# mmammel8/kmer_id

Measured on AMD Instinct MI355X. Metric: paired reads classified/sec on bact10 DB, higher is better.
Workload: dtype u64

## Files before the change

include/kmer_id_amd_bench.h:

```cpp
#ifndef KMER_ID_AMD_BENCH_H
#define KMER_ID_AMD_BENCH_H
#include <stdint.h>
#ifdef __cplusplus
extern "C" {
#endif
struct kid_db;
struct kid_sample;
int kid_synth_db_keys_host(uint64_t seed, int k, const uint64_t *cum, int32_t ntar,
                           uint64_t j0, uint64_t n, uint64_t *keys, uint32_t *targets);
int kid_synth_db_keys_device(uint64_t seed, int k, const uint64_t *cum_host, int32_t ntar,
                             uint64_t j0, uint64_t n, void *d_keys, void *d_targets, int device);
int kid_synth_reads_host(uint64_t db_seed, uint64_t read_seed, int k, const uint64_t *cum,
                         const int32_t *parent, int32_t ntar, uint64_t r0, uint64_t n_reads,
                         uint32_t read_len, uint8_t *bases);
int kid_synth_reads_device(uint64_t db_seed, uint64_t read_seed, int k, const uint64_t *cum_host,
                           const int32_t *parent_host, int32_t ntar, uint64_t r0, uint64_t n_reads,
                           uint32_t read_len, void *d_bases, int device);

int kid_bench_gather(struct kid_db *db, uint64_t n_loads, int inflight, int iters, float *ms_out, uint64_t *loads_out);

int kid_sample_kernel_variants(struct kid_sample *s, uint64_t *mask);

int kid_sample_log_state(struct kid_sample *s, uint32_t *passes, int *has_log, int *logging);

int kid_dev_alloc(int device, uint64_t nbytes, void **d_ptr);
int kid_dev_free(int device, void *d_ptr);
int kid_dev_upload(int device, void *d_dst, const void *src, uint64_t nbytes);
int kid_dev_download(int device, void *dst, const void *d_src, uint64_t nbytes);
int kid_dev_sync(int device);

#ifdef __cplusplus
}
#endif
#endif
```

kmer_id_amd/_lib.py:

```python
import ctypes as C
import os

from . import _build

c_u8p = C.POINTER(C.c_uint8)
c_u32p = C.POINTER(C.c_uint32)
c_i32p = C.POINTER(C.c_int32)
c_u64p = C.POINTER(C.c_uint64)
c_i64p = C.POINTER(C.c_int64)
c_void_pp = C.POINTER(C.c_void_p)


class KidDbInfo(C.Structure):
    _fields_ = [
        ("ntar", C.c_int32), ("k", C.c_int32), ("log2_slots", C.c_int32), ("max_probes", C.c_int32),
        ("flags", C.c_uint32), ("device", C.c_int32), ("tree_depth", C.c_int32), ("host_built", C.c_int32),
        ("geometry", C.c_int32), ("reserved_", C.c_int32),
        ("n_entries", C.c_uint64), ("n_occupied", C.c_uint64), ("table_bytes", C.c_uint64),
    ]


PROTOTYPES = {
    "kid_strerror": (C.c_char_p, [C.c_int]),
    "kid_last_error": (C.c_char_p, []),
# ... 47 lines not shown
    "kid_db_read_segments_fastq": (C.c_int, [C.c_void_p, C.c_void_p, C.c_uint64, C.c_void_p, C.c_uint64, C.c_uint32, C.c_uint32,
                                             C.c_uint32, C.c_uint32, C.c_void_p, C.c_void_p, C.c_uint64, c_u64p]),
    "kid_db_read_segments_device": (C.c_int, [C.c_void_p, C.c_void_p, C.c_uint64, C.c_void_p, C.c_void_p, C.c_void_p, C.c_uint64,
                                              C.c_uint32, C.c_uint32, C.c_uint32, C.c_uint32, C.c_void_p, C.c_uint64, C.c_void_p,
                                              C.c_void_p, C.c_uint64, C.c_void_p, C.c_void_p, C.c_void_p]),
    "kid_db_read_segments_time": (C.c_int, [C.c_void_p, C.POINTER(C.c_double), c_u64p, c_u64p]),
    "kid_sample_end": (C.c_int, [C.c_void_p, C.c_void_p, C.c_void_p]),
    "kid_sample_end_merged": (C.c_int, [c_void_pp, C.c_int, C.c_void_p, C.c_void_p]),
    "kid_sample_stats": (C.c_int, [C.c_void_p, C.c_void_p]),
    "kid_sample_set_timing": (C.c_int, [C.c_void_p, C.c_int]),
    "kid_sample_kernel_time": (C.c_int, [C.c_void_p, C.POINTER(C.c_double), c_u64p]),
    "kid_sample_kernel_time_device": (C.c_int, [C.c_void_p, C.POINTER(C.c_double), c_u64p]),
    "kid_sample_seen_bytes": (C.c_int, [C.c_void_p, c_u64p]),
    "kid_sample_seen_export": (C.c_int, [C.c_void_p, C.c_uint64, C.c_uint64, C.c_void_p, C.c_int]),
    "kid_sample_seen_or": (C.c_int, [C.c_void_p, C.c_uint64, C.c_uint64, C.c_void_p, C.c_int]),
    "kid_sample_gcount": (C.c_int, [C.c_void_p, C.c_void_p]),
    "kid_sample_ucount_range": (C.c_int, [C.c_void_p, C.c_uint64, C.c_uint64, C.c_void_p]),
    "kid_sample_depth_export": (C.c_int, [C.c_void_p, C.c_uint64, C.c_uint64, C.c_void_p, C.c_int]),
    "kid_sample_depth_add": (C.c_int, [C.c_void_p, C.c_uint64, C.c_uint64, C.c_void_p, C.c_int]),
    "kid_sample_depth_spectrum": (C.c_int, [C.c_void_p, C.c_uint32, C.c_void_p, C.c_void_p, C.c_void_p]),
    "kid_sample_depth_spectrum_merged": (C.c_int, [c_void_pp, C.c_int, C.c_uint32, C.c_void_p, C.c_void_p, C.c_void_p]),
    "kid_db_shared_kmers": (C.c_int, [C.c_void_p, c_void_pp, C.c_int, C.c_int, C.c_void_p]),
    "kid_shared_kmers": (C.c_int, [C.c_int, C.c_void_p, C.c_uint64, C.c_int32, c_void_pp, C.c_int, C.c_int, C.c_void_p]),
    "kid_shared_kmers_time": (C.c_int, [C.POINTER(C.c_double), c_u64p]),
    "kid_synth_db_keys_host": (C.c_int, [C.c_uint64, C.c_int, C.c_void_p, C.c_int32, C.c_uint64, C.c_uint64, C.c_void_p,
                                         C.c_void_p]),
    "kid_synth_db_keys_device": (C.c_int, [C.c_uint64, C.c_int, C.c_void_p, C.c_int32, C.c_uint64, C.c_uint64, C.c_void_p,
                                           C.c_void_p, C.c_int]),
    "kid_synth_reads_host": (C.c_int, [C.c_uint64, C.c_uint64, C.c_int, C.c_void_p, C.c_void_p, C.c_int32, C.c_uint64,
                                       C.c_uint64, C.c_uint32, C.c_void_p]),
    "kid_synth_reads_device": (C.c_int, [C.c_uint64, C.c_uint64, C.c_int, C.c_void_p, C.c_void_p, C.c_int32, C.c_uint64,
                                         C.c_uint64, C.c_uint32, C.c_void_p, C.c_int]),
    "kid_sample_kernel_variants": (C.c_int, [C.c_void_p, c_u64p]),
    "kid_sample_log_state": (C.c_int, [C.c_void_p, c_u32p, C.POINTER(C.c_int), C.POINTER(C.c_int)]),
    "kid_bench_gather": (C.c_int, [C.c_void_p, C.c_uint64, C.c_int, C.c_int, C.POINTER(C.c_float), c_u64p]),
    "kid_dev_alloc": (C.c_int, [C.c_int, C.c_uint64, c_void_pp]),
    "kid_dev_free": (C.c_int, [C.c_int, C.c_void_p]),
    "kid_dev_upload": (C.c_int, [C.c_int, C.c_void_p, C.c_void_p, C.c_uint64]),
    "kid_dev_download": (C.c_int, [C.c_int, C.c_void_p, C.c_void_p, C.c_uint64]),
    "kid_dev_sync": (C.c_int, [C.c_int]),
    "kid_device_mem_info": (C.c_int, [C.c_int, c_u64p, c_u64p]),
    "kid_builder_create": (C.c_int, [C.c_int, C.c_int, C.c_void_p, C.c_int32, C.c_uint64, c_void_pp]),
    "kid_builder_destroy": (None, [C.c_void_p]),
    "kid_builder_add": (C.c_int, [C.c_void_p, C.c_void_p, C.c_uint64, C.c_int32]),
    "kid_builder_remove": (C.c_int, [C.c_void_p, C.c_void_p, C.c_uint64]),
    "kid_builder_set_minct": (C.c_int, [C.c_void_p, C.c_void_p, C.c_int32]),
    "kid_builder_claim": (C.c_int, [C.c_void_p, C.c_void_p, C.c_uint64, C.c_int64, C.c_void_p, C.c_uint64, c_u64p]),
    "kid_builder_size": (C.c_int, [C.c_void_p, c_u64p]),
    "kid_builder_export": (C.c_int, [C.c_void_p, C.c_uint64, C.c_uint64, C.c_void_p]),
    "kid_builder_entropy": (C.c_int, [C.c_void_p, C.c_void_p, C.c_uint64, C.c_void_p]),
    "kid_builder_stats": (C.c_int, [C.c_void_p, C.c_void_p, C.c_void_p]),
}

KID_OPT_INPUTS_READY = 1
KID_OPT_LONG_RECORD_KMERS = 2
KID_OPT_MIN_BASE_QUALITY = 3
KID_OPT_ENTRY_DEPTH = 4
KID_DB_OPT_MIN_BASE_QUALITY = 1
KID_SHARED_MAX_SAMPLES = 64
KID_FLAG_U_IS_T = 1
KID_FLAG_HOST_BUILD = 2
KID_FLAG_REF_GEOMETRY = 4

_lib = None


# ... 45 lines not shown
```

kmer_id_amd/api.py:

```python
import ctypes as C
import struct

import numpy as np

from . import _lib
from ._lib import KidDbInfo, check


def _ptr(a):
    return a.ctypes.data_as(C.c_void_p) if a is not None else None


def _as(a, dtype):
    if a is None:
        return None
    a = np.ascontiguousarray(a, dtype=dtype)
    return a


def _offsets_batch(bases, offsets, start, stop):
    offsets = _as(offsets, np.uint64)
    return _as(bases, np.uint8), offsets, _as(start, np.int32), _as(stop, np.int32), offsets.size - 1


# ... 428 lines not shown
    def gcount(self):
        g = np.empty(self.ntar, np.int64)
        check(self._lib.kid_sample_gcount(self._h, _ptr(g)))
        return g

    def ucount_range(self, slot_begin, slot_end):
        u = np.empty(self.ntar, np.int64)
        check(self._lib.kid_sample_ucount_range(self._h, slot_begin, slot_end, _ptr(u)))
        return u

    def stats(self):
        out = np.zeros(4, np.uint64)
        check(self._lib.kid_sample_stats(self._h, _ptr(out)))
        return {"reads": int(out[0]), "lookups": int(out[1]), "probes": int(out[2]), "hits": int(out[3])}

    def set_timing(self, enabled=True):
        check(self._lib.kid_sample_set_timing(self._h, 1 if enabled else 0))

    def kernel_time(self):
        ms, n = C.c_double(0), C.c_uint64(0)
        check(self._lib.kid_sample_kernel_time(self._h, C.byref(ms), C.byref(n)))
        return ms.value, n.value

    def kernel_time_device(self):
        ms, n = C.c_double(0), C.c_uint64(0)
        check(self._lib.kid_sample_kernel_time_device(self._h, C.byref(ms), C.byref(n)))
        return ms.value, n.value

    def kernel_variants(self):
        m = C.c_uint64(0)
        check(self._lib.kid_sample_kernel_variants(self._h, C.byref(m)))
        return {(b >> 3 & 1, b >> 2 & 1, b >> 1 & 1, 30 if b & 1 else 0, b >> 4) for b in range(64) if m.value >> b & 1}

    def log_state(self):
        passes, has_log, logging = C.c_uint32(0), C.c_int(0), C.c_int(0)
        check(self._lib.kid_sample_log_state(self._h, C.byref(passes), C.byref(has_log), C.byref(logging)))
        return {"passes": passes.value, "has_log": bool(has_log.value), "logging": bool(logging.value)}

    def seen_bytes(self):
        n = C.c_uint64(0)
        check(self._lib.kid_sample_seen_bytes(self._h, C.byref(n)))
        return n.value

    def seen_export(self, byte_off, nbytes, dst_ptr=None, on_device=False):
        if dst_ptr is None:
            buf = np.empty(nbytes, np.uint8)
            check(self._lib.kid_sample_seen_export(self._h, byte_off, nbytes, _ptr(buf), 0))
            return buf
        check(self._lib.kid_sample_seen_export(self._h, byte_off, nbytes, C.c_void_p(dst_ptr), 1 if on_device else 0))
        return None

    def seen_or(self, byte_off, src, nbytes=None, on_device=False):
        if isinstance(src, np.ndarray):
            src = np.ascontiguousarray(src, np.uint8)
            check(self._lib.kid_sample_seen_or(self._h, byte_off, src.size, _ptr(src), 0))
        else:
            check(self._lib.kid_sample_seen_or(self._h, byte_off, nbytes, C.c_void_p(src), 1 if on_device else 0))

    def depth_spectrum(self, bins=256):
        spectrum, ksum, dmax = np.empty((self.ntar, bins), np.uint64), np.empty(self.ntar, np.uint64), np.empty(self.ntar, np.uint32)
        check(self._lib.kid_sample_depth_spectrum(self._h, bins, _ptr(spectrum), _ptr(ksum), _ptr(dmax)))
        return spectrum, ksum, dmax

    def entry_depth(self, begin=0, end=None):
        if end is None:
            end = self.db.info.n_entries
# ... 19 lines not shown
```

kmer_id_amd/csrc/kid_api.hip:

```cpp
#include <hip/hip_runtime.h>
#include <memory>
#include <stdint.h>
#include <string.h>
#include <type_traits>
#include <utility>
#include <vector>

#include "../../include/kmer_id_amd.h"
#include "kid_kernels.hip.h"
#include "kid_build.hip.h"
#include "kid_tile.hip.h"
#include "kid_long.hip.h"
#include "kid_hits.hip.h"
#include "kid_support.hip.h"
#include "kid_segments.hip.h"
#include "kid_mask.hip.h"
#include "kid_depth.hip.h"
#include "kid_shared.hip.h"
#include "kid_api_core.h"
#include "kid_api_db.h"
#include "kid_api_mask.h"
#include "kid_api_hits.h"
#include "kid_api_builder.h"
#include "kid_api_bench.h"
// ... 17 lines not shown
        KidDevBuf long_list;
        KidDevBuf long_plan;
        KidDevBuf rare;
        KidEvent ev_prep;
        KidEvent ev_used;
        hipStream_t used_stream = nullptr;
        bool used_recorded = false;
        bool used = false;
    };
    static const int NSET = 3;
    Scratch sets[NSET];
    uint32_t next_set = 0;
    bool inputs_ready = false;
    int min_base_quality = 0;
    KidDevBuf masked;
    int64_t long_kmers = 65536;
    KidDevBuf rare_fixed;
    struct { uint32_t *out_final = nullptr; uint64_t read0 = 0; uint32_t fixed_len = 0; int32_t fixed_nk = 0; bool valid = false; } fixed_held;
    uint64_t dev_clock_batches = 0;
    KidDevBuf seen_log, seen_log_tail, seen_sorted, log_counts, log_bin_total;
    uint32_t seen_log_cap = 0, log_nbins = 0;
    KidMappedHost log_host_total;
    bool log_dirty = false;
    bool log_off = false;
    uint32_t passes_done = 0;
    uint32_t launches_since_apply = 0;
    uint64_t reads_since_apply = 0;
    double log_entries_per_read = 4.0;
    uint64_t reads_of_last_pass = 0;
    KidDevBuf long_hits, long_tiles;
    bool ended = false;
    uint64_t reads_submitted = 0;
    uint64_t kernel_variants = 0;
    hipStream_t last_stream = nullptr;
    bool has_last_stream = false;
    KidEvent order_ev;
    struct Slot {
        KidDevBuf bases;
        KidDevBuf offsets, start, stop, out;
        KidDevBuf recs;
        KidEvent ev_h2d, ev_done, ev_out;
        std::vector<uint64_t> rel;
        uint64_t ticket = 0;
        bool busy = false;
    };
    static const int NSLOT = 3;
    Slot slots[NSLOT];
    uint64_t next_ticket = 1;

    unsigned long long *stats_p() const { return stats.as<unsigned long long>(); }
    volatile unsigned long long *log_rate() const { return static_cast<volatile unsigned long long *>(log_host_total.p); }
    volatile unsigned int *log_off_flag() const { return reinterpret_cast<volatile unsigned int *>(static_cast<char *>(log_host_total.p) + 8); }
};

extern "C" void kid_sample_destroy(kid_sample *s)
{
    if (!s) return;
    if (s->db) hipSetDevice(s->db->device);
    hipDeviceSynchronize();
    delete s;
}

static int kid_seenlog_point(kid_sample *s, hipStream_t stream);
extern "C" int kid_sample_reset(kid_sample *s)
{
    if (!s) return kid_fail(KID_ERR_ARG, "null sample");
    int rc = kid_use_device(s->db->device);
    if (rc != KID_OK) return rc;
    KID_HIP(hipDeviceSynchronize());
    const size_t nt = (size_t)s->db->info.ntar;
    KID_HIP(hipMemset(s->gcount.p, 0, nt * 8));
    KID_HIP(hipMemset(s->ucount.p, 0, nt * 8));
    KID_HIP(hipMemset(s->stats.p, 0, 256));
    KID_HIP(hipMemset(s->masked.p, 0, 8));
    {
        const unsigned long long never = ~0ull;
        KID_HIP(hipMemcpy(s->stats_p() + 30, &never, 8, hipMemcpyHostToDevice));
    }
    s->dev_clock_batches = 0;
    s->reads_submitted = 0;
    s->ended = false;
    s->kernel_variants = 0;
    if (s->seen_log_tail.p) KID_HIP(hipMemset(s->seen_log_tail.p, 0, KID_LOG_SHARDS * 64));
    if (s->seen_log.p) {
        int rc = kid_seenlog_point(s, nullptr);
        if (rc != KID_OK) return rc;
        *s->log_off_flag() = 0;
        *s->log_rate() = 0;
        s->log_off = false;
        s->passes_done = 0;
        s->log_entries_per_read = 4.0;
    }
    s->log_dirty = false;
    s->launches_since_apply = 0;
    s->reads_since_apply = 0;
    KID_HIP(hipMemset(s->seen.p, 0, s->seen_words * 4));
    if (s->depth.p) KID_HIP(hipMemset(s->depth.p, 0, s->seen_words * 32 * 4));
    KID_HIP(hipDeviceSynchronize());
    return KID_OK;
}

extern "C" int kid_sample_begin(kid_db *db, kid_sample **out)
{
    if (!db || !out) return kid_fail(KID_ERR_ARG, "null argument");
    *out = nullptr;
    int rc = kid_use_device(db->device);
    if (rc != KID_OK) return rc;
    std::unique_ptr<kid_sample, void (*)(kid_sample *)> s(new kid_sample(), kid_sample_destroy);
    s->db = db;
    const size_t nt = (size_t)db->info.ntar;
    s->seen_words = db->seen_bits / 32;
    KID_HIP(s->gcount.alloc(nt * 8));
    KID_HIP(s->ucount.alloc(nt * 8));
    KID_HIP(s->stats.alloc(256));
    KID_HIP(s->masked.alloc(8));
    KID_HIP(s->seen.alloc(s->seen_words * 4));
    KID_HIP(s->stream.create());
    const uint64_t nbins = (db->seen_bits + (1ull << KID_LOG_BIN_BITS) - 1) >> KID_LOG_BIN_BITS;
    if (db->d.minloc && nbins <= 1024) {
        uint64_t total = db->info.n_entries * 2ull;
        if (total < (32ull << 20)) total = 32ull << 20;
        if (total > (128ull << 20)) total = 128ull << 20;
        uint64_t cap = (total / KID_LOG_SHARDS) & ~63ull;
        s->seen_log_cap = (uint32_t)cap;
        s->log_nbins = (uint32_t)nbins;
        KID_HIP(s->seen_log.alloc(cap * KID_LOG_SHARDS * 4));
        KID_HIP(s->seen_sorted.alloc(cap * KID_LOG_SHARDS * 4));
        KID_HIP(s->seen_log_tail.alloc(KID_LOG_SHARDS * 64));
        KID_HIP(s->log_counts.alloc(nbins * KID_LOG_WGS * 4));
        KID_HIP(s->log_bin_total.alloc(nbins * 4));
        KID_HIP(s->log_host_total.alloc(64, hipHostMallocMapped));
        memset(s->log_host_total.p, 0, 64);
    }
    const KidRareArgs ra{s->gcount.as<unsigned long long>(), s->stats_p(), db->d.line_mask, 0u, 0ull, 0ull, 0, 0u, db->d.rows,
                         s->seen.as<uint32_t>(), nullptr, nullptr, s->seen_log.as<uint32_t>(), s->seen_log_tail.as<uint32_t>(),
                         s->seen_log_cap, 0u};
    for (kid_sample::Scratch &sc : s->sets) {
        KID_HIP(sc.rare.alloc(sizeof(ra)));
        KID_HIP(hipMemcpy(sc.rare.p, &ra, sizeof(ra), hipMemcpyHostToDevice));
        KID_HIP(sc.ev_prep.create(hipEventDisableTiming));
        KID_HIP(sc.ev_used.create(hipEventDisableTiming));
    }
    KID_HIP(s->rare_fixed.alloc(sizeof(ra)));
    KID_HIP(hipMemcpy(s->rare_fixed.p, &ra, sizeof(ra), hipMemcpyHostToDevice));
    rc = kid_sample_reset(s.get());
    if (rc != KID_OK) return rc;
    *out = s.release();
// ... 129 lines not shown
        }
        if (sc.used && sc.used_stream != prep_stream) {
            if (sc.used_recorded || hipEventRecord(sc.ev_used.e, sc.used_stream) == hipSuccess) KID_HIP(hipStreamWaitEvent(prep_stream, sc.ev_used.e, 0));
            else {
                (void)hipGetLastError();
                KID_HIP(hipDeviceSynchronize());
            }
        }
        const bool fuse_rebase = prep_stream == stream;
        if (fastq)
            hipLaunchKernelGGL(kid_prepare_fastq_kernel, dim3(kid_grid_for(b.n, 256, db->num_cu * 8)), dim3(256), 0, prep_stream, b.bases,
                               fastq, b.n, db->info.k, desc, const_cast<int32_t *>(b.start), const_cast<int32_t *>(b.stop),
                               b.out_final, stats, gcount, rare, ++s->batch_seq, fuse_rebase ? 1 : 0);
        else
            hipLaunchKernelGGL(kid_prepare_kernel, dim3(kid_grid_for(b.n, 256, db->num_cu * 8)), dim3(256), 0, prep_stream, b, db->info.k,
                               desc, stats, rare, ++s->batch_seq, long_cut, sc.long_list.as<KidLongList>(), fuse_rebase ? 1 : 0);
        if (prep_stream != stream) {
            KID_HIP(hipEventRecord(sc.ev_prep.e, prep_stream));
            KID_HIP(hipStreamWaitEvent(stream, sc.ev_prep.e, 0));
        }
        if (long_cut)
            hipLaunchKernelGGL(kid_long_plan_kernel, dim3(1), dim3(64), 0, stream, sc.long_list.as<KidLongList>(), sc.long_plan.as<KidLongPlan>(),
                               desc, rare, s->batch_seq, (uint64_t)s->long_hits.cap / 4, (uint64_t)s->long_tiles.cap - 16);
    }
    const int block = 512, wpb = block / 64;
    const uint32_t ntar = (uint32_t)db->info.ntar;
    const bool ml = db->d.minloc != 0;
    const int grid = kid_grid_for(b.n, wpb, db->num_cu * 16);
    const uint32_t hist_words32 = (ntar + 3u) & ~3u, hist_words16 = ((ntar + 1u) / 2u + 3u) & ~3u;
    const uint32_t hist_words = ml ? hist_words16 : hist_words32;
    const uint32_t wave_words = ml ? KID_GEN_ML_LDS_WORDS : KID_WAVE_LDS_WORDS;
    const bool hist = (hist_words + wpb * wave_words) * 4u + 32u <= 40u * 1024u;
    const bool hist_pair = (hist_words16 + wpb * KID_PAIR_LDS_WORDS) * 4u + 32u <= 40u * 1024u;
    uint64_t span = b.n;
    if (ml && (hist || hist_pair)) {
        const uint64_t per_wg = (uint64_t)(65535u - 2u * (uint32_t)wpb - 64u * (uint32_t)wpb) * (KID_TAPER + 1u) / (2u * KID_TAPER);
        const uint64_t cap = (uint64_t)grid * ((grid & 1) ? per_wg / 2 : per_wg);
        if (span > cap) span = cap;
    }
    KidSampleDev sd{gcount, seen, stats};
    const bool rows = db->d.rows != nullptr, k30 = db->info.k == 30;
    const int32_t fixed_nk = fixed ? (int32_t)(max_kmers > 0 ? max_kmers : 0) : 0;
    const bool want_pair = ml && (max_kmers < 0 || max_kmers <= 2 * 64);
    const bool want_duo = ml && (max_kmers < 0 || (max_kmers > 2 * 64 && max_kmers <= 4 * 64));
    const bool want_general = !ml || max_kmers < 0 || max_kmers > 4 * 64;
    KidEvent ev0, ev1;
    if (s->timing) {
        KID_HIP(ev0.create());
        KID_HIP(ev1.create());
        KID_HIP(hipEventRecord(ev0.e, stream));
    }
    for (uint64_t r0 = 0; r0 < b.n; r0 += span) {
        const uint64_t cnt = b.n - r0 < span ? b.n - r0 : span;
        KidInput pk{b.bases, fixed ? nullptr : desc + r0, b.out_final ? b.out_final + r0 : nullptr, cnt};
        if (fixed) {
            auto &h = s->fixed_held;
            if (!h.valid || h.out_final != pk.out_final || h.read0 != r0 || h.fixed_len != b.fixed_len || h.fixed_nk != fixed_nk) {
                hipLaunchKernelGGL(kid_rebase_kernel, dim3(1), dim3(64), 0, stream, rare, (const KidReadDesc *)nullptr, pk.out_final,
                                   (unsigned long long)r0, b.fixed_len, fixed_nk, (1ull << 32) | (unsigned long long)fixed_nk);
                h.valid = true; h.out_final = pk.out_final; h.read0 = r0; h.fixed_len = b.fixed_len; h.fixed_nk = fixed_nk;
            }
        } else if (r0 != 0 || prep_stream != stream) {
            hipLaunchKernelGGL(kid_rebase_kernel, dim3(1), dim3(64), 0, stream, rare, pk.desc, pk.out_final, 0ull, 0u, 0, 0ull);
        }
        auto launch = [&](auto pk_mode, bool h) {
            constexpr int PK = decltype(pk_mode)::value;
            kid_lift(rows, [&](auto R) { kid_lift(h, [&](auto H) { kid_lift(ml, [&](auto M) { kid_lift(k30, [&](auto K30) {
                if constexpr (PK == 0 || decltype(M)::value) {
                    constexpr bool r = decltype(R)::value, hh = decltype(H)::value, m = decltype(M)::value;
                    constexpr int KF = decltype(K30)::value ? 30 : 0;
                    const uint32_t hw = hh ? (PK ? hist_words16 : hist_words) : 0u;
                    s->kernel_variants |= 1ull << (PK * 16 | r << 3 | hh << 2 | m << 1 | (KF == 30));
                    hipLaunchKernelGGL((kid_classify_kernel<2, r, hh, m, KF, PK>), dim3(grid), dim3(block),
                                       (hw + (size_t)wpb * (PK ? KID_PAIR_LDS_WORDS : wave_words)) * 4 + 32, stream, db->d, pk, sd, hw,
                                       pk.desc, rare);
                }
            }); }); }); });
        };
        if (want_pair) launch(std::integral_constant<int, 1>{}, hist_pair);
        if (want_duo) launch(std::integral_constant<int, 2>{}, hist_pair);
        if (want_general) launch(std::integral_constant<int, 0>{}, hist);
    }
    if (long_cut) {
        hipLaunchKernelGGL(kid_long_hits_kernel, dim3((unsigned)db->num_cu * 8u), dim3(256), 0, stream, db->d, b.bases,
                           scp->long_plan.as<KidLongPlan>(), s->long_hits.as<uint32_t>(), s->long_tiles.as<uint8_t>(), seen, stats);
        hipLaunchKernelGGL(kid_long_fold_kernel, dim3(KID_LONG_MAX), dim3(256), 0, stream, db->d, scp->long_plan.as<KidLongPlan>(),
                           s->long_hits.as<uint32_t>(), s->long_tiles.as<uint8_t>(), gcount, b.out_final);
    }
    if (s->timing) {
        KID_HIP(hipEventRecord(ev1.e, stream));
        s->timed.emplace_back(std::move(ev0), std::move(ev1));
        s->timed_batches++;
    }
    s->dev_clock_batches++;
    if (scp) {
        scp->used_recorded = prep_stream != stream;
        if (scp->used_recorded) KID_HIP(hipEventRecord(scp->ev_used.e, stream));
        scp->used_stream = stream;
        scp->used = true;
    }
    KID_HIP(hipGetLastError());
    s->reads_submitted += b.n;
    return KID_OK;
}

static int kid_depth_set_option(kid_sample *s, int value);
// ... 5 lines not shown
    case KID_OPT_LONG_RECORD_KMERS:
        if (value < 0) return kid_fail(KID_ERR_ARG, "KID_OPT_LONG_RECORD_KMERS: negative threshold");
        s->long_kmers = value;
        return KID_OK;
    case KID_OPT_MIN_BASE_QUALITY: {
        int rc = kid_mask_check_q(value);
        if (rc == KID_OK) s->min_base_quality = value;
        return rc;
    }
    case KID_OPT_ENTRY_DEPTH: return kid_depth_set_option(s, value);
    default: return kid_fail(KID_ERR_ARG, "unknown option %d", option);
    }
}

static int kid_sample_check_open(const kid_sample *s)
{
    if (s->ended) return kid_fail(KID_ERR_STATE, "classify after kid_sample_end without kid_sample_reset");
    return KID_OK;
}

static int kid_prep_stream_for(kid_sample *s, hipStream_t stream, hipStream_t *out)
{
    *out = stream;
    if (!s->inputs_ready) return KID_OK;
    if (!s->prep_stream.s) KID_HIP(s->prep_stream.create(hipStreamNonBlocking));
    *out = s->prep_stream.s;
    return KID_OK;
}

extern "C" int kid_sample_kernel_variants(kid_sample *s, uint64_t *mask)
{
    if (!s || !mask) return kid_fail(KID_ERR_ARG, "null argument");
    *mask = s->kernel_variants;
    return KID_OK;
}

extern "C" int kid_sample_log_state(kid_sample *s, uint32_t *passes, int *has_log, int *logging)
{
    if (!s || !passes || !has_log || !logging) return kid_fail(KID_ERR_ARG, "null argument");
    int rc = kid_use_device(s->db->device);
    if (rc != KID_OK) return rc;
    KID_HIP(hipDeviceSynchronize());
    *passes = s->passes_done;
    *has_log = s->seen_log.p != nullptr;
    *logging = *has_log && *s->log_off_flag() == 0;
    return KID_OK;
}

extern "C" int kid_sample_set_timing(kid_sample *s, int enabled)
{
    if (!s) return kid_fail(KID_ERR_ARG, "null sample");
    s->timing = enabled != 0;
    return KID_OK;
}

extern "C" int kid_sample_kernel_time(kid_sample *s, double *total_ms, uint64_t *launches)
{
    if (!s || !total_ms || !launches) return kid_fail(KID_ERR_ARG, "null argument");
    int rc = kid_use_device(s->db->device);
    if (rc != KID_OK) return rc;
    KID_HIP(hipDeviceSynchronize());
    double sum = 0;
    for (auto &ev : s->timed) {
        float ms = 0;
        KID_HIP(hipEventElapsedTime(&ms, ev.first.e, ev.second.e));
        sum += ms;
// ... 427 lines not shown
```

kmer_id_amd/csrc/kid_kernels.hip.h:

```cpp
#pragma once
#include <hip/hip_runtime.h>
#include <stdint.h>
#include <type_traits>
#include "kid_common.h"

#define KID_WAVE 64
#define KID_TOMBSTONE_HI 0xFFFFFFFFu
#define KID_SEG_KMERS 960
#define KID_WAVE_LDS_WORDS 104
#define KID_CQ_CAP 192
#define KID_CQ_FLUSH 64
#define KID_PAIR_LDS_WORDS (4 + 3 * KID_CQ_CAP + KID_CQ_CAP / 4 + 64 + 128)
#define KID_TAPER 6u
#define KID_EARLY_MAX 4u
#define KID_EARLY_QN 32u
#define KID_GEN_ML_LDS_WORDS (104 + 3 * KID_CQ_CAP + KID_CQ_CAP / 4 + 64)
#define KID_CLASSIFY_OCC 8
#define KID_CLASSIFY_OCC_DUO_ROWS 4

typedef uint32_t kid_u4 __attribute__((ext_vector_type(4)));
typedef uint32_t kid_u2 __attribute__((ext_vector_type(2)));

__device__ __forceinline__ void kid_store_u32_nowait(uint32_t *p, uint32_t v)
{
// ... 46 lines not shown
#define KID_LONG_MAX 1024u
struct KidLongList {
    uint32_t n;
    uint32_t pad[3];
    struct Item { uint64_t first_base; uint32_t n_kmers; uint32_t read; } e[KID_LONG_MAX];
};
struct KidLongRec {
    uint64_t first_base;
    uint64_t hits_off;
    uint32_t n_kmers;
    uint32_t read;
    uint64_t tile0;
};
struct KidLongPlan {
    uint32_t n_recs;
    uint32_t pad;
    uint64_t n_tiles;
    uint64_t total_kmers;
    KidLongRec recs[KID_LONG_MAX];
};

struct KidInput {
    const uint8_t *bases;
    const KidReadDesc *desc;
    uint32_t *out_final;
    uint64_t n;
};

struct KidSampleDev {
    unsigned long long *gcount;
    uint32_t *seen;
    unsigned long long *stats;
};

struct KidRareArgs {
    unsigned long long *gcount;
    unsigned long long *stats;
    uint32_t line_mask;
    uint32_t fixed_len;
    unsigned long long batch_max;
    unsigned long long read0;
    int32_t fixed_nk;
    uint32_t pad;
    const uint4 *rows;
    uint32_t *seen;
    uint32_t *out_final;
    const void *desc;
    uint32_t *seen_log;
    uint32_t *seen_log_tail;
    uint32_t seen_log_cap;
    uint32_t pad2;
};
#define KID_LOG_SHARDS 64u
#define KID_LOG_NONE 0xFFFFFFFFu
#define KID_LOG_BIN_BITS 18
#define KID_LOG_WGS 1024u

__device__ __forceinline__ uint32_t kid_hdr_cand(const uint4 &h, uint32_t fp)
{
    const uint32_t rep = fp * 0x00010001u, one = 0x00010001u, top = 0x80008000u;
    const uint32_t a = h.x ^ rep, b = h.y ^ rep, c = h.z ^ rep, d = (h.w ^ rep) | 0xFFFF0000u;
    return (((a - one) & ~a) & top) | ((((b - one) & ~b) & top) >> 1) | ((((c - one) & ~c) & top) >> 2) |
           ((((d - one) & ~d) & top) >> 3);
}
__device__ __forceinline__ bool kid_hdr_any(const uint4 &h, uint32_t fp)
{
// ... 191 lines not shown
        desc[r] = d;
        if (d.n_kmers > 0 && (uint32_t)d.n_kmers > mx) mx = (uint32_t)d.n_kmers;
    }
    __shared__ uint32_t s_mx;
    if (threadIdx.x == 0) s_mx = 0;
    __syncthreads();
#pragma unroll
    for (int o = 32; o > 0; o >>= 1) { const uint32_t y = (uint32_t)__shfl_xor((int)mx, o); mx = y > mx ? y : mx; }
    if ((threadIdx.x & 63u) == 0 && mx) atomicMax(&s_mx, mx);
    __syncthreads();
    const bool uniform_batch = !b.offsets && !b.start && !b.stop;
    if (threadIdx.x == 0 && (!uniform_batch || blockIdx.x == 0)) {
        const unsigned long long v = ((unsigned long long)seq << 32) | s_mx;
        if (v > *reinterpret_cast<volatile unsigned long long *>(&rare->batch_max)) atomicMax(&rare->batch_max, v);
    }
    if (bad) atomicAdd(&stats[4], (unsigned long long)bad);
}

__global__ void kid_rebase_kernel(KidRareArgs *rare, const KidReadDesc *desc, uint32_t *out_final, unsigned long long read0,
                                  uint32_t fixed_len, int32_t fixed_nk, unsigned long long batch_max)
{
    kid_rebase(rare, desc, out_final, read0, fixed_len, fixed_nk);
    if (threadIdx.x == 0 && batch_max) rare->batch_max = batch_max;
}

template <int U>
struct KidGroup {
    uint64_t key[U];
    uint32_t hlo[U];
    uint4 hd[U];
    uint32_t fpp;
    bool act[U];
};

template <int U, bool ROWS, bool HIST, bool MINLOC, int KFIX, int PAIRK>
__global__ __launch_bounds__(512, (PAIRK == 2 && ROWS) ? KID_CLASSIFY_OCC_DUO_ROWS : KID_CLASSIFY_OCC) void kid_classify_kernel(const KidDevDb db, const KidInput b, const KidSampleDev s,
                                                            const uint32_t hist_words,
                                                            const KidReadDesc *__restrict__ const descs,
                                                            const KidRareArgs *__restrict__ const rare)
{
    static_assert(!PAIRK || (MINLOC && U == 2), "the pair loop exists for the minimizer-localised table, two windows per lane");
    if (MINLOC) {
        const uint32_t longest = (uint32_t)rare->batch_max;
        const int mode = longest <= (uint32_t)(U * 64) ? 1 : longest <= (uint32_t)(2 * U * 64) ? 2 : 0;
        if (mode != PAIRK) return;
    }
    if (threadIdx.x == 0) atomicMin(&s.stats[30], (unsigned long long)__builtin_amdgcn_s_memrealtime());
    extern __shared__ uint32_t kid_smem[];
    const uint32_t lane = threadIdx.x & 63u;
    const uint32_t wib = (uint32_t)__builtin_amdgcn_readfirstlane((int)(threadIdx.x >> 6));
    const uint32_t wpb = blockDim.x >> 6;
    uint32_t *hist = kid_smem;
    uint32_t *WA = kid_smem + hist_words + wib * (PAIRK ? KID_PAIR_LDS_WORDS : MINLOC ? KID_GEN_ML_LDS_WORDS : KID_WAVE_LDS_WORDS);

    unsigned long long *const WGS = reinterpret_cast<unsigned long long *>(
        kid_smem + hist_words + wpb * (PAIRK ? KID_PAIR_LDS_WORDS : MINLOC ? KID_GEN_ML_LDS_WORDS : KID_WAVE_LDS_WORDS));
    if (threadIdx.x < 4) WGS[threadIdx.x] = 0;
    if (HIST) {
        for (uint32_t i = threadIdx.x; i < hist_words; i += blockDim.x) hist[i] = 0;
    }
    __syncthreads();

    const int k = KFIX ? KFIX : db.k;
    const uint32_t win = (uint32_t)kid_min_window(k);
    const int mlen = kid_min_mlen(k);
    const uint32_t bp_src = ((lane + win - 1u) & 63u) << 2;
// ... 607 lines not shown
            const uint32_t nb2 = (uint32_t)b.n, G = gridDim.x, half = G >> 1, wg = blockIdx.x;
            const uint32_t units = wpb * (KID_TAPER * half + (G - half));
            const uint32_t unit = (nb2 + units - 1u) / units;
            const uint32_t mine = wg < half ? KID_TAPER : 1u;
            const uint64_t ufirst = (uint64_t)wpb * (wg < half ? KID_TAPER * wg : KID_TAPER * half + (wg - half)) + (uint64_t)wib * mine;
            const uint64_t f64 = ufirst * unit;
            duo_first = f64 < nb2 ? (uint32_t)f64 : nb2;
            cnt = nb2 - duo_first < mine * unit ? nb2 - duo_first : mine * unit;
            rd_first = duo_first;
            rd_stride = 1u;
            reads_done = cnt;
        }
        constexpr uint32_t BPL = PAIRK == 1 ? 4u : 8u;
        typedef typename std::conditional<PAIRK == 1, uint32_t, kid_u2>::type Raw;
        const uint32_t lane_off = lane * BPL;
        auto ask_lanes = [&](const uint32_t sh, const uint32_t nk) -> uint64_t {
            const uint32_t nl = nk ? (sh + nk + (uint32_t)k - 1u + BPL - 1u) / BPL : 1u;
            return (1ull << nl) - 1ull;
        };
        uint32_t blk = 0, dv_lo = 0, dv_hn = 0;
        auto load_descs = [&](const uint32_t first, const uint32_t len) {
            KidReadDesc d;
            d.first_base = 0; d.n_kmers = 0; d.pad = 0;
            const uint32_t rr = first + lane;
            const KidReadDesc *const dp = static_cast<const KidReadDesc *>(rare->desc);
            if (lane < len) {
                if (dp) d = dp[rr];
                else { d.first_base = (rare->read0 + rr) * (unsigned long long)rare->fixed_len; d.n_kmers = rare->fixed_nk; }
            }
            dv_lo = (uint32_t)d.first_base;
            dv_hn = ((uint32_t)(d.first_base >> 32) & 0xFFFFu) | ((d.n_kmers > 0 ? (uint32_t)d.n_kmers : 0u) << 16);
            if (PAIRK == 1 && lane < len) RG[(blk + lane) & 127u] = rr;
        };
        auto issue_words = [&](const uint32_t idx, Raw &x) {
            const uint32_t hn = (uint32_t)__builtin_amdgcn_readlane((int)dv_hn, (int)idx);
            const uint32_t lo = (uint32_t)__builtin_amdgcn_readlane((int)dv_lo, (int)idx);
            const uint64_t w0 = (((uint64_t)(hn & 0xFFFFu) << 32) | lo) >> 4;
            const uint8_t *const p = reinterpret_cast<const uint8_t *>(uniform64((uint64_t)(b.bases + 16ull * w0)));
            const uint64_t lanes = ask_lanes(lo & 15u, (hn >> 16) & 0x7FFFu);
            uint64_t save;
            if constexpr (PAIRK == 1)
                asm volatile("s_mov_b64 %1, exec\n\ts_mov_b64 exec, %4\n\tglobal_load_dword %0, %2, %3\n\ts_mov_b64 exec, %1"
                             : "+v"(x), "=&s"(save) : "v"(lane_off), "s"(p), "s"(lanes) : "memory");
            else
                asm volatile("s_mov_b64 %1, exec\n\ts_mov_b64 exec, %4\n\tglobal_load_dwordx2 %0, %2, %3\n\ts_mov_b64 exec, %1"
                             : "+v"(x), "=&s"(save) : "v"(lane_off), "s"(p), "s"(lanes) : "memory");
        };
        const uint32_t part_c = PAIRK == 1 ? 24u - 8u * (lane & 3u) : 16u - 16u * (lane & 1u);
        auto pack_lanes = [&](const Raw x, const uint32_t sh, const uint32_t nk, uint32_t &wc, uint32_t &wi) -> bool {
            uint32_t c, d0, d1 = 0;
            if constexpr (PAIRK == 1) c = kid_codes4(x, db.u_is_t, d0);
            else c = (kid_codes4(x.x, db.u_is_t, d0) << 8) | kid_codes4(x.y, db.u_is_t, d1);
            c <<= part_c;
            c |= (uint32_t)__builtin_amdgcn_update_dpp(0, (int)c, 0xB1, 0xF, 0xF, false);
            if constexpr (PAIRK == 1) c |= (uint32_t)__builtin_amdgcn_update_dpp(0, (int)c, 0x4E, 0xF, 0xF, false);
            wc = c;
            wi = 0;
            const uint64_t bad = __ballot((d0 | d1) != 0) & ask_lanes(sh, nk);
            if (bad == 0 || nk == 0) return true;
            const uint32_t end = sh + nk + (uint32_t)k - 1u, lf = sh / BPL, ll = (end - 1u) / BPL;
            uint64_t inside = bad & ~((1ull << lf) | (1ull << ll));
            if (inside == 0) {
                auto lane_bytes = [&](const uint32_t l) -> uint64_t {
                    return ((uint64_t)(uint32_t)__builtin_amdgcn_readlane((int)d1, (int)l) << 32) | (uint32_t)__builtin_amdgcn_readlane((int)d0, (int)l);
                };
                const uint64_t all = BPL == 4u ? 0xFFFFFFFFull : ~0ull;
                const uint64_t from = all << (8u * (sh % BPL)), upto = all >> (8u * (BPL - 1u - ((end - 1u) % BPL)));
                inside = lf == ll ? (lane_bytes(lf) & from & upto) : ((lane_bytes(lf) & from) | (lane_bytes(ll) & upto));
            }
            if (inside == 0) return true;
            uint32_t iv = PAIRK == 1 ? kid_inv4(d0) << (4u * (lane & 3u)) : (kid_inv4(d0) | (kid_inv4(d1) << 4)) << (8u * (lane & 1u));
            iv |= (uint32_t)__builtin_amdgcn_update_dpp(0, (int)iv, 0xB1, 0xF, 0xF, false);
            if constexpr (PAIRK == 1) iv |= (uint32_t)__builtin_amdgcn_update_dpp(0, (int)iv, 0x4E, 0xF, 0xF, false);
// ... 30 lines not shown
                kid_u4 hA0 = issue_header(gA, 0), hA1 = issue_header(gA, 1);
                group_front(nullptr, sh, nb, nk, (uint32_t)(U * 64), cl, gB, bad, false, cC, iC);
                kid_u4 hB0 = issue_header(gB, 0), hB1 = issue_header(gB, 1);
                issue_words(i + 2u - blk, xC);
                n_lookups += nk - bad;
                asm volatile("s_waitcnt vmcnt(3)" : "+v"(hA0), "+v"(hA1) : : "memory");
                gA.hd[0] = make_uint4(hA0.x, hA0.y, hA0.z, hA0.w);
                gA.hd[1] = make_uint4(hA1.x, hA1.y, hA1.z, hA1.w);
                bool had = back_deferred(gA, i);
                if (qn >= KID_CQ_FLUSH) resolve_all(i, i & 63u);
                asm volatile("s_waitcnt vmcnt(1)" : "+v"(hB0), "+v"(hB1) : : "memory");
                gB.hd[0] = make_uint4(hB0.x, hB0.y, hB0.z, hB0.w);
                gB.hd[1] = make_uint4(hB1.x, hB1.y, hB1.z, hB1.w);
                had |= back_deferred(gB, i);
                if (!had) commit_zero(i);
                else if (qn >= KID_CQ_FLUSH) resolve_all(i, 0xFFFFFFFFu);
                if (((i + 1u) & 63u) == 0u) {
                    if (qn || cur_tag != 0xFFFFFFFFu) resolve_all(i, 0xFFFFFFFFu);
                    flush_results(i + 1u - 64u, 64u);
                }
            };
            for (uint32_t i = 0; i < cnt; i += 2) {
                duo(i, xA);
                if (i + 1u < cnt) duo(i + 1u, xB);
            }
            if (qn || cur_tag != 0xFFFFFFFFu) resolve_all(cnt - 1u, 0xFFFFFFFFu);
            if (cnt & 63u) flush_results(cnt & ~63u, cnt & 63u);
            asm volatile("s_waitcnt vmcnt(0)" : "+v"(xA), "+v"(xB) : : "memory");
        } else {
        const uint32_t n32 = (uint32_t)b.n;
        uint32_t seq = 0;
        uint32_t blen = 0;
        uint32_t nreal = 0;
        uint32_t sblk = 0;
        auto switch_block = [&]() {
            const uint32_t G = gridDim.x, half = G >> 1, wg = blockIdx.x;
            const uint32_t units = wpb * (KID_TAPER * half + (G - half));
            const uint32_t unit = (((n32 + units - 1u) / units) + 1u) & ~1u;
            const uint32_t mine = wg < half ? KID_TAPER : 1u;
            const uint64_t ufirst = (uint64_t)wpb * (wg < half ? KID_TAPER * wg : KID_TAPER * half + (wg - half)) + (uint64_t)wib * mine;
            const uint64_t wave_first = ufirst * unit, off = (uint64_t)sblk * 64u, wave_cnt = (uint64_t)mine * unit;
            sblk++;
            const uint64_t f64 = wave_first + off;
            const uint32_t first = f64 < n32 ? (uint32_t)f64 : n32;
            uint32_t len = off < wave_cnt ? (uint32_t)(wave_cnt - off < 64u ? wave_cnt - off : 64u) : 0u;
            if (len > n32 - first) len = n32 - first;
            load_descs(first, len);
            blen = len;
        };
        switch_block();
        bool more = blen != 0;
        if (more) {
            issue_words(0u, xA);
            issue_words(1u, xB);
        }
        while (more) {
            const uint32_t i = seq;
            const uint32_t ia = i - blk;
            const uint32_t hnA = (uint32_t)__builtin_amdgcn_readlane((int)dv_hn, (int)ia), hnB = (uint32_t)__builtin_amdgcn_readlane((int)dv_hn, (int)(ia + 1u));
            const uint32_t nkA = (hnA >> 16) & 0x7FFFu, nkB = (hnB >> 16) & 0x7FFFu;
            const uint32_t shA = (uint32_t)__builtin_amdgcn_readlane((int)dv_lo, (int)ia) & 15u;
            const uint32_t shB = (uint32_t)__builtin_amdgcn_readlane((int)dv_lo, (int)(ia + 1u)) & 15u;
            const bool realB = ia + 1u < blen;
            KidGroup<U> gA, gB;
            uint32_t badA = 0, badB = 0;
            if (ia + 2u >= blen) {
                blk = i + 2u;
                switch_block();
                more = blen != 0;
            }

            asm volatile("s_waitcnt vmcnt(1)" : "+v"(xA) : : "memory");
            uint32_t cA, iA;
            const bool clA = pack_lanes(xA, shA, nkA, cA, iA);
            group_front(nullptr, shA, nkA + (uint32_t)k - 1, nkA, 0u, clA, gA, badA, false, cA, iA);
            kid_u4 hA0 = issue_header(gA, 0), hA1 = issue_header(gA, 1);
            issue_words(i + 2u - blk, xA);

            asm volatile("s_waitcnt vmcnt(3)" : "+v"(xB) : : "memory");
            uint32_t cB, iB;
            const bool clB = pack_lanes(xB, shB, nkB, cB, iB);
            group_front(nullptr, shB, nkB + (uint32_t)k - 1, nkB, 0u, clB, gB, badB, false, cB, iB);
            kid_u4 hB0 = issue_header(gB, 0), hB1 = issue_header(gB, 1);
            issue_words(i + 3u - blk, xB);

            asm volatile("s_waitcnt vmcnt(4)" : "+v"(hA0), "+v"(hA1) : : "memory");
            gA.hd[0] = make_uint4(hA0.x, hA0.y, hA0.z, hA0.w);
            gA.hd[1] = make_uint4(hA1.x, hA1.y, hA1.z, hA1.w);
            n_lookups += nkA - badA;
            if (!back_deferred(gA, i)) commit_zero(i);
            else if (qn >= KID_CQ_FLUSH) resolve_all(i, 0xFFFFFFFFu);

            asm volatile("s_waitcnt vmcnt(1)" : "+v"(hB0), "+v"(hB1) : : "memory");
            gB.hd[0] = make_uint4(hB0.x, hB0.y, hB0.z, hB0.w);
            gB.hd[1] = make_uint4(hB1.x, hB1.y, hB1.z, hB1.w);
            nreal += realB ? 2u : 1u;
            if (realB) {
                n_lookups += nkB - badB;
                if (!back_deferred(gB, i + 1u)) commit_zero(i + 1u);
                else if (qn >= KID_CQ_FLUSH) resolve_all(i + 1u, 0xFFFFFFFFu);
            }
            seq = i + 2u;
            if ((seq & 63u) == 0u) {
                if (qn) resolve_all(i + 1u, 0xFFFFFFFFu);
                flush_results(seq - 64u, 64u);
            }
        }
        asm volatile("s_waitcnt vmcnt(0)" : "+v"(xA), "+v"(xB) : : "memory");
        if (nreal & 1u) seq -= 1u;
        reads_done = seq;
        if (qn) resolve_all(seq - 1u, 0xFFFFFFFFu);
        if (seq & 63u) flush_results(seq & ~63u, seq & 63u);
        }
    }
    if constexpr (PAIRK == 0) {
        const uint32_t n32 = (uint32_t)b.n;
        gen_cnt = gw32 < n32 ? (n32 - gw32 + nw32 - 1u) / nw32 : 0u;
        if (MINLOC) {
            const uint32_t G = gridDim.x, half = G >> 1, wg = blockIdx.x;
            const uint32_t units = wpb * (KID_TAPER * half + (G - half));
            const uint32_t unit = (n32 + units - 1u) / units;
            const uint32_t mine = wg < half ? KID_TAPER : 1u;
            const uint64_t ufirst = (uint64_t)wpb * (wg < half ? KID_TAPER * wg : KID_TAPER * half + (wg - half)) + (uint64_t)wib * mine;
            const uint64_t f64 = ufirst * unit;
            rd_first = f64 < n32 ? (uint32_t)f64 : n32;
            rd_stride = 1u;
            gen_cnt = n32 - rd_first < mine * unit ? n32 - rd_first : mine * unit;
            reads_done = gen_cnt;
        }
        const uint32_t gf = rd_first, gs = rd_stride, gc = gen_cnt;
        KidReadDesc dA, dB;
        kid_u4 xA, xB;
        fetch_desc(gc > 0u ? gf : n32, dA);
        fetch_desc(gc > 1u ? gf + gs : n32, dB);
        fetch_words(dA, xA);
        for (uint32_t i = 0; i < gc; i += 2) {
            const uint32_t r = gf + i * gs;
            short_read(r, i, uniform64(dA.first_base), __builtin_amdgcn_readfirstlane(dA.n_kmers), xA,
                       [&]() { fetch_words(dB, xB); fetch_desc(i + 2u < gc ? r + 2u * gs : n32, dA); });
            if (i + 1u >= gc) break;
            short_read(r + gs, i + 1u, uniform64(dB.first_base), __builtin_amdgcn_readfirstlane(dB.n_kmers), xB,
                       [&]() { fetch_words(dA, xA); fetch_desc(i + 3u < gc ? r + 3u * gs : n32, dB); });
            if (MINLOC && ((i + 2u) & 63u) == 0u) {
// ... 31 lines not shown
    if (HIST) {
        __syncthreads();
        for (uint32_t i = threadIdx.x; i < hist_words; i += blockDim.x) {
            const uint32_t v = hist[i];
            if (MINLOC) {
                if (v & 0xFFFFu) atomicAdd(&rare->gcount[2u * i], (unsigned long long)(v & 0xFFFFu));
                if (v >> 16) atomicAdd(&rare->gcount[2u * i + 1u], (unsigned long long)(v >> 16));
            } else if (v) atomicAdd(&rare->gcount[i], (unsigned long long)v);
        }
    }
    if (lane == 0) {
        const unsigned long long tl = *WL, n_reads = reads_done;
        const uint32_t n_hits = WC[2];
        const unsigned long long te = WC[3];
        if (n_reads) atomicAdd(&WGS[0], n_reads);
        if (tl) atomicAdd(&WGS[1], tl);
        if (tl + te) atomicAdd(&WGS[2], tl + te);
        if (n_hits) atomicAdd(&WGS[3], (unsigned long long)n_hits);
    }
    __syncthreads();
    if (threadIdx.x < 4) {
        const unsigned long long v = WGS[threadIdx.x];
        if (v) atomicAdd(&rare->stats[threadIdx.x], v);
    }
    if (threadIdx.x == 0) {
        unsigned long long prev = atomicMax(&s.stats[31], (unsigned long long)__builtin_amdgcn_s_memrealtime());
        asm volatile("" : "+v"(prev));
        unsigned long long done = atomicAdd(&s.stats[29], 1ull);
        if (done + 1ull == (unsigned long long)gridDim.x) {
            const unsigned long long a = atomicAdd(&s.stats[30], 0ull), z = atomicAdd(&s.stats[31], 0ull);
            if (z > a) { atomicAdd(&s.stats[6], z - a); atomicAdd(&s.stats[7], 1ull); }
            unsigned long long t0 = atomicExch(&s.stats[30], ~0ull), t1 = atomicExch(&s.stats[31], 0ull);
            asm volatile("" : "+v"(t0), "+v"(t1));
            atomicExch(&s.stats[29], 0ull);
        }
    }
}

__global__ void kid_lookup_kernel(const KidDevDb db, const uint64_t *keys, uint64_t n, uint32_t *targets, uint32_t *probes)
{
    for (uint64_t i = blockIdx.x * (uint64_t)blockDim.x + threadIdx.x; i < n; i += (uint64_t)gridDim.x * blockDim.x) {
        uint32_t slot, np;
        targets[i] = kid_dev_lookup(db, keys[i], slot, np);
        if (probes) probes[i] = np;
    }
}

__global__ void kid_fmix_kernel(const uint64_t *keys, uint64_t n, uint64_t *out)
{
    for (uint64_t i = blockIdx.x * (uint64_t)blockDim.x + threadIdx.x; i < n; i += (uint64_t)gridDim.x * blockDim.x)
        out[i] = kid_fmix64(keys[i]);
}

__global__ void kid_msca_kernel(const KidDevDb db, const int32_t *x, const int32_t *y, uint64_t n, int32_t *out)
{
    for (uint64_t i = blockIdx.x * (uint64_t)blockDim.x + threadIdx.x; i < n; i += (uint64_t)gridDim.x * blockDim.x) {
        const uint32_t a = (uint32_t)x[i], c = (uint32_t)y[i];
        uint32_t r;
        if (db.rows) {
            uint4 ro;
            r = kid_msca_rows(a, db.rows[a], c, db.rows[c], ro);
        } else {
            r = kid_msca_climb(db, a, c);
        }
        out[i] = (int32_t)r;
    }
// ... 419 lines not shown
```

Measured before the change: 1.178 billion.

## Use dynamic work-stealing blocks and occupancy-sized grid for paired classify kernel

Replaces the static tapered per-wave read partition in the paired classify kernel with a global atomic counter that hands out read blocks of geometrically shrinking size, which reduces tail imbalance between waves. The paired kernel's grid is now sized from queried occupancy per CU instead of sharing the general grid, with an optional user cap. This adds a global atomic per block fetch and resets the counter at kernel end. It also enlarges the stats buffer and issues the first two text loads together.

```diff
diff --git a/include/kmer_id_amd_bench.h b/include/kmer_id_amd_bench.h
--- a/include/kmer_id_amd_bench.h
+++ b/include/kmer_id_amd_bench.h
@@ -21,6 +21,8 @@
 
 int kid_sample_kernel_variants(struct kid_sample *s, uint64_t *mask);
 
+int kid_sample_set_classify_grid(struct kid_sample *s, int workgroups);
+
 int kid_sample_log_state(struct kid_sample *s, uint32_t *passes, int *has_log, int *logging);
 
 int kid_dev_alloc(int device, uint64_t nbytes, void **d_ptr);
diff --git a/kmer_id_amd/_lib.py b/kmer_id_amd/_lib.py
--- a/kmer_id_amd/_lib.py
+++ b/kmer_id_amd/_lib.py
@@ -103,6 +103,7 @@
     "kid_synth_reads_device": (C.c_int, [C.c_uint64, C.c_uint64, C.c_int, C.c_void_p, C.c_void_p, C.c_int32, C.c_uint64,
                                          C.c_uint64, C.c_uint32, C.c_void_p, C.c_int]),
     "kid_sample_kernel_variants": (C.c_int, [C.c_void_p, c_u64p]),
+    "kid_sample_set_classify_grid": (C.c_int, [C.c_void_p, C.c_int]),
     "kid_sample_log_state": (C.c_int, [C.c_void_p, c_u32p, C.POINTER(C.c_int), C.POINTER(C.c_int)]),
     "kid_bench_gather": (C.c_int, [C.c_void_p, C.c_uint64, C.c_int, C.c_int, C.POINTER(C.c_float), c_u64p]),
     "kid_dev_alloc": (C.c_int, [C.c_int, C.c_uint64, c_void_pp]),
diff --git a/kmer_id_amd/api.py b/kmer_id_amd/api.py
--- a/kmer_id_amd/api.py
+++ b/kmer_id_amd/api.py
@@ -484,6 +484,9 @@
         check(self._lib.kid_sample_kernel_variants(self._h, C.byref(m)))
         return {(b >> 3 & 1, b >> 2 & 1, b >> 1 & 1, 30 if b & 1 else 0, b >> 4) for b in range(64) if m.value >> b & 1}
 
+    def set_classify_grid(self, workgroups):
+        check(self._lib.kid_sample_set_classify_grid(self._h, int(workgroups)))
+
     def log_state(self):
         passes, has_log, logging = C.c_uint32(0), C.c_int(0), C.c_int(0)
         check(self._lib.kid_sample_log_state(self._h, C.byref(passes), C.byref(has_log), C.byref(logging)))
diff --git a/kmer_id_amd/csrc/kid_api.hip b/kmer_id_amd/csrc/kid_api.hip
--- a/kmer_id_amd/csrc/kid_api.hip
+++ b/kmer_id_amd/csrc/kid_api.hip
@@ -73,6 +73,8 @@
     bool ended = false;
     uint64_t reads_submitted = 0;
     uint64_t kernel_variants = 0;
+    int classify_grid = 0;
+    int pair_resident[8] = {};
     hipStream_t last_stream = nullptr;
     bool has_last_stream = false;
     KidEvent order_ev;
@@ -112,7 +114,7 @@
     const size_t nt = (size_t)s->db->info.ntar;
     KID_HIP(hipMemset(s->gcount.p, 0, nt * 8));
     KID_HIP(hipMemset(s->ucount.p, 0, nt * 8));
-    KID_HIP(hipMemset(s->stats.p, 0, 256));
+    KID_HIP(hipMemset(s->stats.p, 0, KID_STATS_BYTES));
     KID_HIP(hipMemset(s->masked.p, 0, 8));
     {
         const unsigned long long never = ~0ull;
@@ -153,7 +155,7 @@
     s->seen_words = db->seen_bits / 32;
     KID_HIP(s->gcount.alloc(nt * 8));
     KID_HIP(s->ucount.alloc(nt * 8));
-    KID_HIP(s->stats.alloc(256));
+    KID_HIP(s->stats.alloc(KID_STATS_BYTES));
     KID_HIP(s->masked.alloc(8));
     KID_HIP(s->seen.alloc(s->seen_words * 4));
     KID_HIP(s->stream.create());
@@ -349,18 +351,38 @@
     const uint32_t wave_words = ml ? KID_GEN_ML_LDS_WORDS : KID_WAVE_LDS_WORDS;
     const bool hist = (hist_words + wpb * wave_words) * 4u + 32u <= 40u * 1024u;
     const bool hist_pair = (hist_words16 + wpb * KID_PAIR_LDS_WORDS) * 4u + 32u <= 40u * 1024u;
+    const bool rows = db->d.rows != nullptr, k30 = db->info.k == 30;
+    const bool want_pair = ml && (max_kmers < 0 || max_kmers <= 2 * 64);
+    const bool want_duo = ml && (max_kmers < 0 || (max_kmers > 2 * 64 && max_kmers <= 4 * 64));
+    const bool want_general = !ml || max_kmers < 0 || max_kmers > 4 * 64;
+    int grid_pair = 0;
+    const size_t lds_pair = ((hist_pair ? hist_words16 : 0u) + (size_t)wpb * KID_PAIR_LDS_WORDS) * 4 + 32;
+    if (want_pair) {
+        int &res = s->pair_resident[(rows ? 4 : 0) | (hist_pair ? 2 : 0) | (k30 ? 1 : 0)];
+        if (res == 0) {
+            int occ = 0;
+            kid_lift(rows, [&](auto R) { kid_lift(hist_pair, [&](auto H) { kid_lift(k30, [&](auto K30) {
+                (void)hipOccupancyMaxActiveBlocksPerMultiprocessor(
+                    &occ, kid_classify_kernel<2, decltype(R)::value, decltype(H)::value, true, decltype(K30)::value ? 30 : 0, 1>, block, lds_pair);
+            }); }); });
+            if (occ < 1) { (void)hipGetLastError(); occ = 1; }
+            res = occ;
+        }
+        grid_pair = kid_grid_for(b.n, 2 * wpb, db->num_cu * res);
+        if (s->classify_grid > 0 && grid_pair > s->classify_grid) grid_pair = s->classify_grid;
+    }
     uint64_t span = b.n;
-    if (ml && (hist || hist_pair)) {
+    if (want_pair && hist_pair) {
+        const uint64_t cap = (uint64_t)grid_pair * (65535u - 64u * (uint32_t)wpb);
+        if (span > cap) span = cap;
+    }
+    if (ml && ((want_duo && hist_pair) || (want_general && hist))) {
         const uint64_t per_wg = (uint64_t)(65535u - 2u * (uint32_t)wpb - 64u * (uint32_t)wpb) * (KID_TAPER + 1u) / (2u * KID_TAPER);
         const uint64_t cap = (uint64_t)grid * ((grid & 1) ? per_wg / 2 : per_wg);
         if (span > cap) span = cap;
     }
     KidSampleDev sd{gcount, seen, stats};
-    const bool rows = db->d.rows != nullptr, k30 = db->info.k == 30;
     const int32_t fixed_nk = fixed ? (int32_t)(max_kmers > 0 ? max_kmers : 0) : 0;
-    const bool want_pair = ml && (max_kmers < 0 || max_kmers <= 2 * 64);
-    const bool want_duo = ml && (max_kmers < 0 || (max_kmers > 2 * 64 && max_kmers <= 4 * 64));
-    const bool want_general = !ml || max_kmers < 0 || max_kmers > 4 * 64;
     KidEvent ev0, ev1;
     if (s->timing) {
         KID_HIP(ev0.create());
@@ -388,7 +410,7 @@
                     constexpr int KF = decltype(K30)::value ? 30 : 0;
                     const uint32_t hw = hh ? (PK ? hist_words16 : hist_words) : 0u;
                     s->kernel_variants |= 1ull << (PK * 16 | r << 3 | hh << 2 | m << 1 | (KF == 30));
-                    hipLaunchKernelGGL((kid_classify_kernel<2, r, hh, m, KF, PK>), dim3(grid), dim3(block),
+                    hipLaunchKernelGGL((kid_classify_kernel<2, r, hh, m, KF, PK>), dim3(PK == 1 ? grid_pair : grid), dim3(block),
                                        (hw + (size_t)wpb * (PK ? KID_PAIR_LDS_WORDS : wave_words)) * 4 + 32, stream, db->d, pk, sd, hw,
                                        pk.desc, rare);
                 }
@@ -460,6 +482,14 @@
 {
     if (!s || !mask) return kid_fail(KID_ERR_ARG, "null argument");
     *mask = s->kernel_variants;
+    return KID_OK;
+}
+
+extern "C" int kid_sample_set_classify_grid(kid_sample *s, int workgroups)
+{
+    if (!s) return kid_fail(KID_ERR_ARG, "null sample");
+    if (workgroups < 0) return kid_fail(KID_ERR_ARG, "kid_sample_set_classify_grid: negative grid");
+    s->classify_grid = workgroups;
     return KID_OK;
 }
 
diff --git a/kmer_id_amd/csrc/kid_kernels.hip.h b/kmer_id_amd/csrc/kid_kernels.hip.h
--- a/kmer_id_amd/csrc/kid_kernels.hip.h
+++ b/kmer_id_amd/csrc/kid_kernels.hip.h
@@ -102,6 +102,8 @@
     uint32_t *seen;
     unsigned long long *stats;
 };
+#define KID_STATS_HEAD 32
+#define KID_STATS_BYTES 384
 
 struct KidRareArgs {
     unsigned long long *gcount;
@@ -359,6 +361,33 @@
     uint32_t fpp;
     bool act[U];
 };
+
+__device__ __forceinline__ void kid_block_of(uint32_t t, const uint32_t n, const uint32_t nw, uint32_t &first, uint32_t &len)
+{
+    uint32_t ls = 6u;
+    while (ls > 1u && (n >> ls) < nw) ls--;
+    const uint32_t l1 = ls > 2u ? ls - 1u : 1u, l2 = ls > 3u ? ls - 2u : 1u, l3 = ls > 4u ? ls - 3u : 1u;
+    const uint32_t h = nw >> 1;
+    const uint32_t tail = (h << l1) + (h << l2) + (nw << l3);
+    const uint32_t nb0 = n > tail ? (n - tail + (1u << ls) - 1u) >> ls : 0u;
+    uint64_t f;
+    uint32_t l = ls;
+    if (t < nb0) f = (uint64_t)t << ls;
+    else {
+        t -= nb0;
+        f = (uint64_t)nb0 << ls;
+        if (t < h) { f += (uint64_t)t << l1; l = l1; }
+        else {
+            t -= h;
+            f += (uint64_t)h << l1;
+            if (t < h) { f += (uint64_t)t << l2; l = l2; }
+            else { f += ((uint64_t)h << l2) + ((uint64_t)(t - h) << l3); l = l3; }
+        }
+    }
+    first = f < n ? (uint32_t)f : n;
+    len = 1u << l;
+    if (len > n - first) len = n - first;
+}
 
 template <int U, bool ROWS, bool HIST, bool MINLOC, int KFIX, int PAIRK>
 __global__ __launch_bounds__(512, (PAIRK == 2 && ROWS) ? KID_CLASSIFY_OCC_DUO_ROWS : KID_CLASSIFY_OCC) void kid_classify_kernel(const KidDevDb db, const KidInput b, const KidSampleDev s,
@@ -1032,13 +1061,16 @@
             dv_hn = ((uint32_t)(d.first_base >> 32) & 0xFFFFu) | ((d.n_kmers > 0 ? (uint32_t)d.n_kmers : 0u) << 16);
             if (PAIRK == 1 && lane < len) RG[(blk + lane) & 127u] = rr;
         };
-        auto issue_words = [&](const uint32_t idx, Raw &x) {
+        auto text_of = [&](const uint32_t idx, uint64_t &lanes) -> const uint8_t * {
             const uint32_t hn = (uint32_t)__builtin_amdgcn_readlane((int)dv_hn, (int)idx);
             const uint32_t lo = (uint32_t)__builtin_amdgcn_readlane((int)dv_lo, (int)idx);
             const uint64_t w0 = (((uint64_t)(hn & 0xFFFFu) << 32) | lo) >> 4;
-            const uint8_t *const p = reinterpret_cast<const uint8_t *>(uniform64((uint64_t)(b.bases + 16ull * w0)));
-            const uint64_t lanes = ask_lanes(lo & 15u, (hn >> 16) & 0x7FFFu);
-            uint64_t save;
+            lanes = ask_lanes(lo & 15u, (hn >> 16) & 0x7FFFu);
+            return reinterpret_cast<const uint8_t *>(uniform64((uint64_t)(b.bases + 16ull * w0)));
+        };
+        auto issue_words = [&](const uint32_t idx, Raw &x) {
+            uint64_t lanes, save;
+            const uint8_t *const p = text_of(idx, lanes);
             if constexpr (PAIRK == 1)
                 asm volatile("s_mov_b64 %1, exec\n\ts_mov_b64 exec, %4\n\tglobal_load_dword %0, %2, %3\n\ts_mov_b64 exec, %1"
                              : "+v"(x), "=&s"(save) : "v"(lane_off), "s"(p), "s"(lanes) : "memory");
@@ -1135,27 +1167,33 @@
         uint32_t seq = 0;
         uint32_t blen = 0;
         uint32_t nreal = 0;
-        uint32_t sblk = 0;
-        auto switch_block = [&]() {
-            const uint32_t G = gridDim.x, half = G >> 1, wg = blockIdx.x;
-            const uint32_t units = wpb * (KID_TAPER * half + (G - half));
-            const uint32_t unit = (((n32 + units - 1u) / units) + 1u) & ~1u;
-            const uint32_t mine = wg < half ? KID_TAPER : 1u;
-            const uint64_t ufirst = (uint64_t)wpb * (wg < half ? KID_TAPER * wg : KID_TAPER * half + (wg - half)) + (uint64_t)wib * mine;
-            const uint64_t wave_first = ufirst * unit, off = (uint64_t)sblk * 64u, wave_cnt = (uint64_t)mine * unit;
-            sblk++;
-            const uint64_t f64 = wave_first + off;
-            const uint32_t first = f64 < n32 ? (uint32_t)f64 : n32;
-            uint32_t len = off < wave_cnt ? (uint32_t)(wave_cnt - off < 64u ? wave_cnt - off : 64u) : 0u;
-            if (len > n32 - first) len = n32 - first;
+        auto switch_block = [&](const bool first_block) {
+            const uint32_t nw32 = gridDim.x * wpb;
+            uint32_t t = (uint32_t)gw;
+            bool take = true;
+            if (!first_block) {
+                const uint32_t have = (uint32_t)__builtin_amdgcn_readfirstlane(
+                    (int)*static_cast<volatile uint32_t *>(kid_smem + hist_words + wpb * KID_PAIR_LDS_WORDS));
+                take = have + 64u * wpb <= 65535u;
+                uint32_t drawn = 0;
+                if (take && lane == 0) drawn = atomicAdd(reinterpret_cast<uint32_t *>(s.stats + KID_STATS_HEAD), 1u);
+                t = nw32 + (uint32_t)__builtin_amdgcn_readfirstlane((int)drawn);
+            }
+            uint32_t first, len;
+            kid_block_of(t, n32, nw32, first, len);
+            if (!take) len = 0;
+            if (len && lane == 0) atomicAdd(&WGS[0], (unsigned long long)len);
             load_descs(first, len);
             blen = len;
         };
-        switch_block();
+        switch_block(true);
         bool more = blen != 0;
         if (more) {
-            issue_words(0u, xA);
-            issue_words(1u, xB);
+            uint64_t lanesA, lanesB, save;
+            const uint8_t *const pA = text_of(0u, lanesA), *const pB = text_of(1u, lanesB);
+            asm volatile("s_mov_b64 %2, exec\n\ts_mov_b64 exec, %6\n\tglobal_load_dword %0, %3, %4\n\ts_mov_b64 exec, %7\n\t"
+                         "global_load_dword %1, %3, %5\n\ts_mov_b64 exec, %2\n\ts_waitcnt vmcnt(0)"
+                         : "+v"(xA), "+v"(xB), "=&s"(save) : "v"(lane_off), "s"(pA), "s"(pB), "s"(lanesA), "s"(lanesB) : "memory");
         }
         while (more) {
             const uint32_t i = seq;
@@ -1169,7 +1207,7 @@
             uint32_t badA = 0, badB = 0;
             if (ia + 2u >= blen) {
                 blk = i + 2u;
-                switch_block();
+                switch_block(false);
                 more = blen != 0;
             }
 
@@ -1211,7 +1249,7 @@
         }
         asm volatile("s_waitcnt vmcnt(0)" : "+v"(xA), "+v"(xB) : : "memory");
         if (nreal & 1u) seq -= 1u;
-        reads_done = seq;
+        reads_done = 0u;
         if (qn) resolve_all(seq - 1u, 0xFFFFFFFFu);
         if (seq & 63u) flush_results(seq & ~63u, seq & 63u);
         }
@@ -1309,6 +1347,10 @@
             if (z > a) { atomicAdd(&s.stats[6], z - a); atomicAdd(&s.stats[7], 1ull); }
             unsigned long long t0 = atomicExch(&s.stats[30], ~0ull), t1 = atomicExch(&s.stats[31], 0ull);
             asm volatile("" : "+v"(t0), "+v"(t1));
+            if (PAIRK == 1) {
+                uint32_t h = atomicExch(reinterpret_cast<uint32_t *>(s.stats + KID_STATS_HEAD), 0u);
+                asm volatile("" : "+v"(h));
+            }
             atomicExch(&s.stats[29], 0ull);
         }
     }
```

Measured after the change: 1.012 billion. 0.859x the previous value.
